# syghmon/bridges-with-reinforcement-learning

Hardware: AMD Instinct MI355X
Metric: env-steps/sec (vectorised assembly_gym, tower_height=4) (higher is better)
Workload: dtype f64

## Files before the change

### bridges-with-reinforcement-learning_amd/csrc/env_kernels.hip

```cpp
#include "bridges_device.h"
#include "rbe_device.h"

namespace bridges {

__device__ inline void reset_env(const DevCtx& c, int e, int lane) {
    c.b.state_bits[(size_t)e * IMG + lane] = 0ull;
    if (lane < c.K) c.b.blk_occ[(size_t)e * c.K + lane] = 0;
    if (lane == 0) {
        c.b.n_blocks[e] = 0;
        c.b.n_if[e] = 0;
        c.b.targets_left[e] = (c.n_targets >= 32) ? 0xffffffffu : ((1u << c.n_targets) - 1u);
        c.b.needs_reset[e] = 0;
    }
}

__device__ inline int count_candidates(const DevCtx& c, int e, int nb, int lane) {
    int nfree = 0;
    for (int i0 = 0; i0 < nb * MAXV; i0 += WAVE) {
        int i = i0 + lane;
        bool fr = false;
        if (i < nb * MAXV) {
            int b = i / MAXV, f = i % MAXV;
            int nv = c.tt->shapes[c.b.blk_shape[(size_t)e * c.K + b]].nv;
            fr = f < nv && !((c.b.blk_occ[(size_t)e * c.K + b] >> f) & 1);
        }
        nfree += __popcll(__ballot(fr));
    }
    return c.n_groups * (c.n_ground + nfree * c.n_offsets);
}

__global__ __launch_bounds__(WAVE) void k_reset(DevCtx c) {
    int e = blockIdx.x, lane = threadIdx.x;
    reset_env(c, e, lane);
    if (lane < 8) c.b.step_flags[(size_t)e * 8 + lane] = 0;
    int nc = count_candidates(c, e, 0, lane);
    if (lane == 0) {
        c.b.reward[e] = 0.f;
        c.b.lin_reward[e] = 0.f;
        c.b.n_reached[e] = 0;
        c.b.draw_counter[e] = 0;
        c.b.n_cand[e] = nc;
    }
}

#define STEP_IF_LDS 32
#define STEP_TAB_LDS 4096
struct StepStage {
    bridges_shape shapes[8];
    double pose[MAXK * 4];
    double verts[MAXK * MAXV * 2];
    int32_t shape_id[MAXK];
    int32_t occ[MAXK];
};
struct StepKeep {
    double if_geom[STEP_IF_LDS * 8];
    int32_t if_body[STEP_IF_LDS * 2];
    double cen[MAXK * 2];
    double vol[MAXK];
};
static_assert(sizeof(StepStage) <= STEP_TAB_LDS * sizeof(double), "staging area must fit into the tableau storage");

__device__ __forceinline__ const double* step_targets() { return nullptr; }
__device__ __forceinline__ const double* step_targets(const double* p) { return p; }
template <typename... ENV_TARGETS>
__global__ __launch_bounds__(WAVE) void k_step(DevCtx c, ENV_TARGETS... env_targets_arg) {
    constexpr bool PER_ENV = sizeof...(ENV_TARGETS) == 1;
    const double* env_targets = step_targets(env_targets_arg...);
    (void)env_targets;
    __shared__ __attribute__((aligned(16))) double tab[STEP_TAB_LDS];
    __shared__ LpScratch S;
    __shared__ StepKeep Lk;
    StepStage& L = *reinterpret_cast<StepStage*>(tab);
    __builtin_amdgcn_s_setprio(3);
    const int e = blockIdx.x, lane = threadIdx.x;
    const int K = c.K;
    uint8_t* flags = c.b.step_flags + (size_t)e * 8;
    int32_t* shape_id_g = c.b.blk_shape + (size_t)e * K;
    double* pose_g = c.b.blk_pose + (size_t)e * K * 4;
    double* verts_g = c.b.blk_verts + (size_t)e * K * MAXV * 2;
    uint8_t* occ_g = c.b.blk_occ + (size_t)e * K;
    int32_t* if_body_g = c.b.if_body + (size_t)e * MAXIF * 2;
    double* if_geom_g = c.b.if_geom + (size_t)e * MAXIF * 8;
    double* ws = c.b.lp_ws + (size_t)e * c.b.lp_ws_stride;
    const WarmHdr* hdr_g = reinterpret_cast<const WarmHdr*>(ws);

    const uint8_t need_reset = c.b.needs_reset[e];
    const int a = c.b.sel_index[e];
    const int off = c.b.cand_offset[e];
    const int nb = c.b.n_blocks[e];
    const int n_if_old = c.b.n_if[e];
    uint32_t left = c.b.targets_left[e];
    const uint64_t sbits = c.b.state_bits[(size_t)e * IMG + lane];
    WarmPre W;
    W.magic = hdr_g->magic; W.n_blocks = hdr_g->n_blocks; W.n_if = hdr_g->n_if; W.stride = hdr_g->stride;
    W.half = hdr_g->half; W.m = hdr_g->m;
    W.basis_lane = hdr_g->basis[lane];
    double tgv = 0.0;
    if constexpr (PER_ENV) {
        if (lane < c.n_targets * 3) tgv = env_targets[(size_t)e * c.n_targets * 3 + lane];
    }
    {
        const double* src = reinterpret_cast<const double*>(c.tt->shapes);
        double* dst = reinterpret_cast<double*>(L.shapes);
        const int nd = c.n_shapes * (int)(sizeof(bridges_shape) / 8);
        for (int i = lane; i < nd; i += WAVE) dst[i] = src[i];
        for (int i = lane; i < nb * 4; i += WAVE) L.pose[i] = pose_g[i];
        for (int i = lane; i < nb * MAXV * 2; i += WAVE) L.verts[i] = verts_g[i];
        if (lane < K) { L.shape_id[lane] = shape_id_g[lane]; L.occ[lane] = occ_g[lane]; }
        const int n0 = n_if_old < STEP_IF_LDS ? n_if_old : STEP_IF_LDS;
        for (int i = lane; i < n0 * 8; i += WAVE) Lk.if_geom[i] = if_geom_g[i];
        for (int i = lane; i < n0 * 2; i += WAVE) Lk.if_body[i] = if_body_g[i];
    }

    if (need_reset) {
        reset_env(c, e, lane);
        if (lane < 8) flags[lane] = 0;
        if (lane == 0) {
            c.b.reward[e] = 0.f;
            c.b.lin_reward[e] = 0.f;
            c.b.n_reached[e] = 0;
        }
        if (lane == 0) c.b.n_cand[e] = c.n_groups * c.n_ground;
        return;
    }

    const size_t ci = (size_t)off + a;
    const int dsc = lane < 4 ? c.b.cand_desc[ci * 4 + lane] : 0;
    const double cpose = lane < 4 ? c.b.cand_pose[ci * 4 + lane] : 0.0;
    const double cvert = lane < MAXV * 2 ? c.b.cand_verts[ci * MAXV * 2 + lane] : 0.0;
    const uint64_t cbits = c.b.cand_bits[ci * IMG + lane];
    const float base = c.b.cand_lin[ci];
    warm_prefetch(W, ws, nb, n_if_old, lane);
    const int tb = __builtin_amdgcn_readlane(dsc, 0), tf = __builtin_amdgcn_readlane(dsc, 1);
    const int sh = __builtin_amdgcn_readlane(dsc, 2), fc = __builtin_amdgcn_readlane(dsc, 3);

    if (lane < 4) { L.pose[nb * 4 + lane] = cpose; pose_g[nb * 4 + lane] = cpose; }
    if (lane < MAXV * 2) { L.verts[nb * MAXV * 2 + lane] = cvert; verts_g[nb * MAXV * 2 + lane] = cvert; }
    c.b.state_bits[(size_t)e * IMG + lane] = sbits | cbits;
    __syncthreads();
    if (lane == 0) {
        L.shape_id[nb] = sh;
        shape_id_g[nb] = sh;
        L.occ[nb] = (int32_t)(1u << fc);
        occ_g[nb] = (uint8_t)(1u << fc);
        if (tb >= 0) {
            L.occ[tb] |= (int32_t)(1u << tf);
            occ_g[tb] = (uint8_t)L.occ[tb];
        }
        c.b.n_blocks[e] = nb + 1;
    }
    __syncthreads();
    const bridges_shape* shapes = L.shapes;
    const bridges_shape& shn = shapes[sh];
    int nf = 0;
    if (lane <= nb) {
        const bridges_shape& sb = shapes[L.shape_id[lane]];
        double rgx, rgz;
        rot2(sb.gx, sb.gz, L.pose[4 * lane + 2], L.pose[4 * lane + 3], rgx, rgz);
        Lk.cen[2 * lane] = L.pose[4 * lane] + rgx;
        Lk.cen[2 * lane + 1] = L.pose[4 * lane + 1] + rgz;
        Lk.vol[lane] = sb.volume;
        nf = sb.nv - __popc((uint32_t)L.occ[lane] & ((1u << sb.nv) - 1u));
    }

    double vx = 0.0, vz = 0.0;
    const int nvn = shn.nv;
    bool hasv = lane < nvn;
    if (hasv) { vx = L.verts[nb * MAXV * 2 + 2 * lane]; vz = L.verts[nb * MAXV * 2 + 2 * lane + 1]; }
    double x0 = wave_min_d(hasv ? vx : 1e300), x1 = wave_max_d(hasv ? vx : -1e300);
    double z0 = wave_min_d(hasv ? vz : 1e300), z1 = wave_max_d(hasv ? vz : -1e300);
    {
        double cx = (x0 + x1) * 0.5, cz = (z0 + z1) * 0.5, hx = (x1 - x0) * 0.5, hz = (z1 - z0) * 0.5;
        double hy = shn.depth * 0.5;
        bool skip = false;
        for (int t = 0; t < c.n_targets; ++t) {
            if (!((left >> t) & 1u)) continue;
            if (skip) { skip = false; continue; }
            bool in;
            if constexpr (PER_ENV) {
                const double tx = readlane_d(tgv, 3 * t), ty = readlane_d(tgv, 3 * t + 1), tz = readlane_d(tgv, 3 * t + 2);
                in = fabs(tx - cx) < hx + 1e-6 && fabs(ty) < hy + 1e-6 && fabs(tz - cz) < hz + 1e-6;
            } else {
                in = fabs(c.targets[t][0] - cx) < hx + 1e-6 && fabs(c.targets[t][1]) < hy + 1e-6 &&
                     fabs(c.targets[t][2] - cz) < hz + 1e-6;
            }
            if (in) { left &= ~(1u << t); skip = true; }
        }
    }
    const int n_reached = c.n_targets - __popc(left);

    int n_if = n_if_old;
    bool overflow = false;
    {
        const double* nverts = L.verts + nb * MAXV * 2;
        const int totalp = (1 + nb * MAXV) * MAXV;
        for (int p0 = 0; p0 < totalp; p0 += WAVE) {
            const int p = p0 + lane;
            bool hit = false;
            double g[8];
            int bodyA = -1;
            if (p < totalp) {
                const int qa = p / MAXV, fn = p % MAXV;
                if (fn < shn.nv) {
                    const int ia = shn.fa[fn], ib = shn.fb[fn];
                    const double aBx = nverts[2 * ia], aBz = nverts[2 * ia + 1], bBx = nverts[2 * ib], bBz = nverts[2 * ib + 1];
                    const Frame2 fB = edge_frame(aBx, aBz, bBx, bBz);
                    if (qa == 0) {
                        hit = face_pair_contact_v(-c.floor_hw, 0.0, c.floor_hw, 0.0, 0.0, 0.0, 1.0, 0.0, 0.0, 1.0, aBx, aBz, bBx,
                                                  bBz, fB.cx, fB.cz, fB.nx, fB.nz, fmin(c.floor_depth, shn.depth), g);
                    } else {
                        bodyA = (qa - 1) / MAXV;
                        const int f = (qa - 1) % MAXV;
                        const bridges_shape& sa = shapes[L.shape_id[bodyA]];
                        if (f < sa.nv) {
                            const double* v = L.verts + bodyA * MAXV * 2;
                            const double ax = v[2 * sa.fa[f]], az = v[2 * sa.fa[f] + 1], bx = v[2 * sa.fb[f]], bz = v[2 * sa.fb[f] + 1];
                            const Frame2 fr = edge_frame(ax, az, bx, bz);
                            hit = face_pair_contact_v(ax, az, bx, bz, fr.cx, fr.cz, fr.tx, fr.tz, fr.nx, fr.nz, aBx, aBz, bBx, bBz,
                                                      fB.cx, fB.cz, fB.nx, fB.nz, fmin(sa.depth, shn.depth), g);
                        }
                    }
                }
            }
            const uint64_t bal = __ballot(hit);
            const int idx = n_if + __popcll(bal & ((1ull << lane) - 1ull));
            if (hit && idx < MAXIF) {
                if_body_g[2 * idx] = bodyA;
                if_body_g[2 * idx + 1] = nb;
#pragma unroll
                for (int k = 0; k < 8; ++k) if_geom_g[8 * idx + k] = g[k];
                if (idx < STEP_IF_LDS) {
                    Lk.if_body[2 * idx] = bodyA;
                    Lk.if_body[2 * idx + 1] = nb;
#pragma unroll
                    for (int k = 0; k < 8; ++k) Lk.if_geom[8 * idx + k] = g[k];
                }
            }
            n_if += __popcll(bal);
        }
        if (n_if > MAXIF) { overflow = true; n_if = MAXIF; }
    }
    __syncthreads();

    bool err = false;
    bool st_frozen = true, st_free = true;
    bool warm_used = false, resolved = false;
    AsmView A;
    A.pose = nullptr; A.shape_id = nullptr; A.shapes = nullptr; A.n_blocks = nb + 1;
    A.cand_b = -1; A.cand_pose = nullptr; A.cand_shape = 0; A.cen = Lk.cen; A.vol = Lk.vol; A.n_tens = 0; A.tens_coef = 1.0;
    A.n_if = n_if; A.n_if0 = n_if < STEP_IF_LDS ? n_if : STEP_IF_LDS;
    A.if_body0 = Lk.if_body; A.if_geom0 = Lk.if_geom;
    A.if_body1 = if_body_g + 2 * STEP_IF_LDS; A.if_geom1 = if_geom_g + 8 * STEP_IF_LDS;
    rbe_both(tab, STEP_TAB_LDS, ws, c.b.lp_ws_stride, S, A, n_if_old, W, c.mu, c.density, lane, &st_frozen, &st_free, &err,
             &warm_used, c.b.lp_snap ? c.b.lp_snap + (size_t)e * c.b.lp_snap_stride : nullptr, &resolved);

    const bool all_reached = left == 0;
    const bool terminated = !st_frozen || all_reached;
    const bool truncated = (c.max_steps > 0 && (nb + 1) >= c.max_steps) || (nb + 1) >= K;
    const bool done = terminated || truncated;
    float reward = !st_frozen ? -1.f : (all_reached ? (float)n_reached : (float)(-1 + n_reached));
    float lin = st_free ? base : (st_frozen ? base / 100.f : 0.f);

    if (lane == 0) {
        flags[F_VALID] = 1; flags[F_STABLE_FROZEN] = st_frozen; flags[F_STABLE_UNFROZEN] = st_free;
        flags[F_TERMINATED] = terminated; flags[F_TRUNCATED] = truncated; flags[F_DONE] = done;
        flags[F_NO_ACTIONS] = 0; flags[F_LP_ERROR] = (uint8_t)((err ? 1 : 0) | (overflow ? 2 : 0) | (resolved ? 4 : 0));
        c.b.reward[e] = reward;
        c.b.lin_reward[e] = lin;
        c.b.n_reached[e] = n_reached;
        c.b.n_if[e] = n_if;
        c.b.targets_left[e] = left;
    }
    int nb_after = nb + 1;
    if (done) {
        reset_env(c, e, lane);
        nb_after = 0;
    }
    int nfree = 0;
    for (int b = 0; b < nb_after; ++b) nfree += __builtin_amdgcn_readlane(nf, b);
    const int nc = c.n_groups * (c.n_ground + nfree * c.n_offsets);
    if (lane == 0) c.b.n_cand[e] = nc;
}

#define SCAN_THREADS 256
#define SCAN_WAVES (SCAN_THREADS / WAVE)
#define SCAN_BATCH 8
__global__ __launch_bounds__(SCAN_THREADS) void k_scan(DevCtx c, int after_step) {
    __shared__ int wave_tot[SCAN_WAVES];
    __shared__ int carry_s;
    __shared__ unsigned long long red[SCAN_WAVES][8];
    __builtin_amdgcn_s_setprio(3);
    const int t = threadIdx.x, lane = t & 63, wv = t >> 6;
    if (t == 0) carry_s = 0;
    __syncthreads();
    unsigned long long acc[8] = {0, 0, 0, 0, 0, 0, 0, 0};
    for (int base0 = 0; base0 < c.E; base0 += SCAN_THREADS * SCAN_BATCH) {
        int v[SCAN_BATCH], nbk[SCAN_BATCH], nval[SCAN_BATCH];
        uint64_t fl8[SCAN_BATCH];
#pragma unroll
        for (int u = 0; u < SCAN_BATCH; ++u) {
            const int i = base0 + u * SCAN_THREADS + t;
            const bool in = i < c.E;
            v[u] = in ? c.b.n_cand[i] : 0;
            nbk[u] = in ? c.b.n_blocks[i] : 0;
            nval[u] = (in && after_step) ? c.b.n_valid[i] : 0;
            fl8[u] = (in && after_step) ? *reinterpret_cast<const uint64_t*>(c.b.step_flags + (size_t)i * 8) : 0ull;
        }
#pragma unroll
        for (int u = 0; u < SCAN_BATCH; ++u) {
            const int base = base0 + u * SCAN_THREADS;
            if (base >= c.E) break;
            const int i = base + t;
            if (i < c.E) {
                if (v[u] > c.a_max) {
                    v[u] = c.a_max;
                    c.b.n_cand[i] = c.a_max;
                    c.b.step_flags[(size_t)i * 8 + F_LP_ERROR] |= 8;
                    acc[7] += 1;
                }
                acc[0] += (unsigned long long)nbk[u];
                if (after_step) {
                    const unsigned valid = (unsigned)(fl8[u] >> (8 * F_VALID)) & 0xffu;
                    const unsigned lperr = (unsigned)(fl8[u] >> (8 * F_LP_ERROR)) & 0xffu;
                    acc[1] += valid ? 1 : 0;
                    acc[2] += valid ? 0 : 1;
                    acc[3] += (lperr & 1) ? 1 : 0;
                    acc[4] += (lperr & 2) ? 1 : 0;
                    acc[5] += (unsigned long long)nval[u];
                    acc[6] += (lperr & 4) ? 1 : 0;
                }
            }
            int incl = v[u];
#pragma unroll
            for (int o = 1; o < WAVE; o <<= 1) {
                int up = __shfl_up(incl, o, WAVE);
                if (lane >= o) incl += up;
            }
            if (lane == WAVE - 1) wave_tot[wv] = incl;
            __syncthreads();
            int wbase = 0;
            for (int k = 0; k < wv; ++k) wbase += wave_tot[k];
            const int carry = carry_s;
            if (i < c.E) c.b.cand_offset[i] = carry + wbase + incl - v[u];
            __syncthreads();
            if (t == SCAN_THREADS - 1) carry_s = carry + wbase + incl;
            __syncthreads();
        }
    }
#pragma unroll
    for (int k = 0; k < 8; ++k) {
        unsigned long long x = acc[k];
#pragma unroll
        for (int o = 32; o > 0; o >>= 1) x += __shfl_xor(x, o, WAVE);
        if (lane == 0) red[wv][k] = x;
    }
    __syncthreads();
    if (t == 0) {
        unsigned long long tot[8] = {0, 0, 0, 0, 0, 0, 0, 0};
        for (int w = 0; w < SCAN_WAVES; ++w)
            for (int k = 0; k < 8; ++k) tot[k] += red[w][k];
        c.b.cand_offset[c.E] = carry_s;
        if (c.h_total) *c.h_total = carry_s;
        c.b.stats[ST_SUM_CAND] += (uint64_t)carry_s;
        c.b.stats[ST_SUM_BLOCKS] += tot[0];
        c.b.stats[ST_ENV_STEPS] += tot[1];
        c.b.stats[ST_RESET_ONLY] += tot[2];
        c.b.stats[ST_LP_ERRORS] += tot[3];
        c.b.stats[ST_IF_OVERFLOW] += tot[4];
        c.b.stats[ST_SUM_VALID] += tot[5];
        c.b.stats[ST_WARM_RESOLVED] += tot[6];
        c.b.stats[ST_CAND_OVERFLOW] += tot[7];
        c.b.stats[ST_LOCKSTEPS] += 1;
    }
}

__global__ __launch_bounds__(WAVE) void k_enumerate(DevCtx c) {
    __shared__ uint8_t free_b[MAXK * MAXV], free_f[MAXK * MAXV];
    __shared__ bridges_shape sh_l[8];
    __shared__ double verts_l[MAXK * MAXV * 2];
    __shared__ int32_t shape_l[MAXK], occ_l[MAXK];
    __shared__ double xg_l[32], offs_l[8];
    __builtin_amdgcn_s_setprio(3);
    const int e = blockIdx.x, lane = threadIdx.x;
    const int K = c.K;
    if (lane < 32) xg_l[lane] = c.tt->x_ground[lane];
    if (lane < 8) offs_l[lane] = c.tt->offsets[lane];
    const int nb = c.b.n_blocks[e];
    const int ncand = c.b.n_cand[e];
    const size_t off = (size_t)c.b.cand_offset[e];
    {
        const double* src = reinterpret_cast<const double*>(c.tt->shapes);
        double* dst = reinterpret_cast<double*>(sh_l);
        const int nd = c.n_shapes * (int)(sizeof(bridges_shape) / 8);
        for (int i = lane; i < nd; i += WAVE) dst[i] = src[i];
        const double* vg = c.b.blk_verts + (size_t)e * K * MAXV * 2;
        for (int i = lane; i < nb * MAXV * 2; i += WAVE) verts_l[i] = vg[i];
        if (lane < K) { shape_l[lane] = c.b.blk_shape[(size_t)e * K + lane]; occ_l[lane] = c.b.blk_occ[(size_t)e * K + lane]; }
    }
    __syncthreads();
    const bridges_shape* shapes = sh_l;
    const int32_t* shape_id = shape_l;
    const double* verts = verts_l;
    int nfree = 0;
    for (int i0 = 0; i0 < nb * MAXV; i0 += WAVE) {
        int i = i0 + lane;
        bool fr = false;
// ... 747 lines not shown
```

### bridges-with-reinforcement-learning_amd/csrc/rbe_device.h

```cpp
#pragma once
#include "bridges_device.h"

namespace bridges {

#define RBE_TOL_PARALLEL 1e-6
#define RBE_TOL_COPLANAR 1e-6
#define RBE_AMIN 0.001
#define RBE_FEAS_TOL 1e-5
#define LP_EPS_COST 1e-9
#define LP_TAU 1e-5
#define LP_VERIFY_TOL 1e-4
#define LP_TIE 1e-9
#define LP_STALL 40
#define LP_MAX_PIVOTS 5000
#define LP_PERTURB 1e-8
#define LP_MARGIN 1e3
#define LP_MARGIN_LO 0.1
#define LP_S_MAX 1e4
#define LP_TAB_LDS 2048
#define MAXFACES (1 + MAXK * MAXV)
#define LP_MAX_COLS (4 * MAXIF)
#define LP_MAX_CHUNKS ((LP_MAX_COLS + 2 + WAVE - 1) / WAVE)

struct FaceLds {
// ... 330 lines not shown
                for (int u = 0; u < 4; ++u) {
                    if (idx + u * WAVE < cells) {
                        double v;
                        if (ii[u] == r) v = rv[u];
                        else if (qq[u] == jin) v = 0.0;
                        else v = tv[u] - cv[u] * rv[u];
                        T[ii[u] * stride + qq[u]] = v;
                    }
                }
            }
        }
        if (lane == 0) basis[r] = jin;
        wave_sync<IN_LDS>();
        const double wn = -T[mc * stride + n];
        if (wn < w - progress) { stall = 0; bland = false; }
        else if (++stall > LP_STALL) bland = true;
        w = wn;
        if (++pivots >= LP_MAX_PIVOTS) { *error = true; w = artificial_sum(T, stride, m, n, basis, lane); break; }
    }
    *pivots_out = pivots;
    return w;
}

template <typename TP, typename SC>
__device__ inline double lp_verify(TP T, int stride, int m, int m_chk, int n, SC& S, const AsmView& A, double mu,
                                   double density, int lane) {
    for (int q = lane; q < n; q += WAVE) S.rowr[q] = 0.0;
    __syncthreads();
    if (lane <= m && S.basis[lane] >= 0 && S.basis[lane] < n) {
        double v = T[lane * stride + n + 1];
        S.rowr[S.basis[lane]] = v > 0.0 ? v : 0.0;
    }
    __syncthreads();
    double res = 0.0;
    if (lane < m_chk && S.basis[lane] != -1) {
        int b = -1;
        for (int k = 0; k < A.n_blocks; ++k) if (S.row_of[k] >= 0 && S.row_of[k] <= lane && lane < S.row_of[k] + 3) b = k;
        const int comp = lane - S.row_of[b];
        double gcx, gcz;
        A.centroid(b, gcx, gcz);
        double acc = 0.0;
        for (int k = 0; k < A.n_if; ++k) {
            const int32_t* bd = A.ib(k);
            const int bA = bd[0], bB = bd[1];
            if (bA != b && bB != b) continue;
            const double sign = (bB == b) ? 1.0 : -1.0;
            const double* g = A.ig(k);
#pragma unroll
            for (int c4 = 0; c4 < 4; ++c4) {
                const int ip = c4 >> 1, ig = c4 & 1;
                const double x = S.rowr[4 * k + c4];
                if (x == 0.0) continue;
                const double px = ip ? g[2] : g[0], pz = ip ? g[3] : g[1];
                const double gx = sign * (ig ? g[4] - mu * g[6] : g[4] + mu * g[6]);
                const double gz = sign * (ig ? g[5] - mu * g[7] : g[5] + mu * g[7]);
                const double coef = comp == 0 ? gx : (comp == 1 ? gz : (px - gcx) * gz - (pz - gcz) * gx);
                acc += coef * x;
            }
            if (A.n_tens) {
#pragma unroll
                for (int ip = 0; ip < 2; ++ip) {
                    const double x = S.rowr[4 * A.n_if + 2 * k + ip];
                    if (x == 0.0) continue;
                    const double px = ip ? g[2] : g[0], pz = ip ? g[3] : g[1];
                    const double gx = -sign * g[4], gz = -sign * g[5];
                    const double coef = comp == 0 ? gx : (comp == 1 ? gz : (px - gcx) * gz - (pz - gcz) * gx);
                    acc += coef * x;
                }
            }
        }
        const double rhs = comp == 1 ? density * A.volume(b) : 0.0;
        res = fabs(acc - rhs);
    }
    return wave_sum_d(res);
}

template <bool IN_LDS, typename TP, typename SC>
__device__ inline void lp_activate_rows(TP T, int stride, int m, int m_act, int n_gen, SC& S, int lane, int ncarr = 0) {
    const int n = n_gen + 1;
    for (int i = m_act; i < m; ++i) {
        const bool neg = T[i * stride + n] < 0.0;
        wave_sync<IN_LDS>();
        for (int q = lane; q <= n + ncarr; q += WAVE) {
            double v = T[i * stride + q];
            if (neg) { v = -v; T[i * stride + q] = v; }
            T[(m + 1) * stride + q] -= v;
        }
        if (lane == 0) S.basis[i] = n + i;
    }
    wave_sync<IN_LDS>();
}

template <typename SC>
__device__ inline void lp_row_map(SC& S, uint32_t free_mask, int lane) {
    __syncthreads();
    if (lane < MAXK)
        S.row_of[lane] = ((free_mask >> lane) & 1u) ? 3 * __popc(free_mask & ((1u << lane) - 1u)) : -1;
    __syncthreads();
}

__device__ __forceinline__ void lp_dims(int n_free, int n_if, int& m, int& n, int& stride, int64_t& cells, bool carriers = false,
                                        int n_tens = 0) {
    m = 3 * n_free;
    n = 4 * n_if + 2 * n_tens;
    stride = n + 2 + (carriers ? m : 0);
    if ((stride & 1) == 0) stride += 1;
    cells = (int64_t)(m + 2) * stride;
}

template <typename SC>
__device__ inline bool rbe_stable(double* tab_lds, int lds_cap, int max_cols, double* tab_ws, int64_t ws_cap, SC& S,
                                  const AsmView& A, uint32_t fixed_mask, double mu, double density, int lane,
                                  double* w_out, int* pivots_out, bool* error, bool* too_big) {
    *w_out = 0.0;
    *pivots_out = 0;
    const int n_blocks = A.n_blocks;
    const uint32_t all = n_blocks >= 32 ? 0xffffffffu : ((1u << n_blocks) - 1u);
    const uint32_t free_mask = all & ~fixed_mask;
    const int n_free = __popc(free_mask);
    if (A.n_if == 0) return n_free == 0;
    if (n_free == 0) return true;
    int m, n, stride;
    int64_t cells;
    lp_dims(n_free, A.n_if, m, n, stride, cells, false, A.n_tens);
    const double feas = RBE_FEAS_TOL * density, vtol = LP_VERIFY_TOL * density;
    double w;
    if (cells <= lds_cap && n <= max_cols) {
        lp_row_map(S, free_mask, lane);
        lp_build(tab_lds, stride, m, m, n, A, S.row_of, mu, density, lane);
        w = lp_phase1<true>(tab_lds, stride, m, m, n, S, lane, pivots_out, error, true, feas);
        if (w <= feas && lp_verify(tab_lds, stride, m, m, n, S, A, mu, density, lane) > vtol) { *error = true; w = 1e300; }
    } else {
        if (cells > ws_cap || n > max_cols) { *too_big = true; return false; }
        lp_row_map(S, free_mask, lane);
        lp_build(tab_ws, stride, m, m, n, A, S.row_of, mu, density, lane);
        w = lp_phase1<false>(tab_ws, stride, m, m, n, S, lane, pivots_out, error, true, feas);
        if (w <= feas && lp_verify(tab_ws, stride, m, m, n, S, A, mu, density, lane) > vtol) { *error = true; w = 1e300; }
    }
    *w_out = w;
    return w <= feas;
}

#define WARM_HDR_DOUBLES 64
#define WARM_MAX_STRIDE (LP_MAX_COLS + 2 + 3 * MAXK + 1)
#define WARM_HALF ((int64_t)(3 * MAXK + 2) * WARM_MAX_STRIDE)
#define WARM_WS_DOUBLES (WARM_HDR_DOUBLES + 2 * WARM_HALF)
#define WARM_MAGIC 0x57A7B1E5

struct WarmHdr {
    int32_t magic, n_blocks, n_if, stride, half, m, pad_[10];
    int32_t basis[64];
};

#define WARM_PRE 16
struct WarmPre {
    int32_t magic, n_blocks, n_if, stride, half, m;
    int32_t basis_lane;
    bool ok;
    int n_pre;
    double cell[WARM_PRE];
};

__device__ __forceinline__ void warm_header(WarmPre& W, const double* ws, int lane) {
    const WarmHdr* h = reinterpret_cast<const WarmHdr*>(ws);
    W.magic = h->magic; W.n_blocks = h->n_blocks; W.n_if = h->n_if; W.stride = h->stride; W.half = h->half; W.m = h->m;
    W.basis_lane = h->basis[lane];
}

__device__ __forceinline__ bool warm_matches(const WarmPre& W, int n_old_blocks, int n_if_old) {
    return W.magic == WARM_MAGIC && W.n_blocks == n_old_blocks && W.n_if == n_if_old && n_old_blocks >= 1 &&
           W.m == 3 * n_old_blocks;
}

__device__ __forceinline__ void warm_prefetch(WarmPre& W, const double* ws, int n_old_blocks, int n_if_old, int lane) {
    W.ok = warm_matches(W, n_old_blocks, n_if_old);
    W.n_pre = WARM_PRE;
    const int m_o = 3 * n_old_blocks, ncols_o = 4 * n_if_old + 2 + m_o;
    const int cells_o = W.ok ? (m_o + 1) * ncols_o : 0;
    const double* src = ws + WARM_HDR_DOUBLES + (int64_t)(W.half & 1) * WARM_HALF;
    const int di = WAVE / ncols_o, dq = WAVE - di * ncols_o;
    int i = lane / ncols_o, q = lane - i * ncols_o;
#pragma unroll
    for (int u = 0; u < WARM_PRE; ++u) {
        const int idx = lane + WAVE * u;
        double v = 0.0;
        if (idx < cells_o) v = src[(size_t)i * W.stride + q];
        W.cell[u] = v;
        i += di; q += dq;
        if (q >= ncols_o) { q -= ncols_o; ++i; }
    }
}

template <bool IN_LDS, typename TP, typename SC>
__device__ inline void lp_warm_prepare(TP T, int stride, int m, int n_gen, const double* src, int stride_o, int m_o,
                                       int n_gen_o, const WarmPre& W, SC& S, const AsmView& A, double mu,
                                       double density, int lane) {
    const int n = n_gen + 1, n_o = n_gen_o + 1;
    const int ncols_o = n_o + 1 + m_o;
    const int cells = (m + 2) * stride;
    for (int i = lane; i < cells; i += WAVE) T[i] = 0.0;
    wave_sync<IN_LDS>();
    const int cells_o = (m_o + 1) * ncols_o;
    const int di_o = WAVE / ncols_o, dq_o = WAVE - di_o * ncols_o;
    int ci_o = lane / ncols_o, cq_o = lane - ci_o * ncols_o;
#pragma unroll
    for (int u = 0; u < WARM_PRE; ++u) {
        const int idx = lane + WAVE * u;
        if (u < W.n_pre && idx < cells_o) {
            const int i = ci_o, q = cq_o;
            const int qn = q < n_gen_o ? q : (q == n_gen_o ? n_gen : (q == n_o ? n : n + 1 + (q - n_o - 1)));
            const int in = i < m_o ? i : m;
            T[in * stride + qn] = W.cell[u];
        }
        if (u < W.n_pre) {
            ci_o += di_o; cq_o += dq_o;
            if (cq_o >= ncols_o) { cq_o -= ncols_o; ++ci_o; }
        }
    }
    for (int idx = lane + WAVE * W.n_pre; idx < cells_o; idx += WAVE) {
        const int i = ci_o, q = cq_o;
        const double v = src[(size_t)i * stride_o + q];
        const int qn = q < n_gen_o ? q : (q == n_gen_o ? n_gen : (q == n_o ? n : n + 1 + (q - n_o - 1)));
        const int in = i < m_o ? i : m;
        T[in * stride + qn] = v;
        ci_o += di_o; cq_o += dq_o;
        if (cq_o >= ncols_o) { cq_o -= ncols_o; ++ci_o; }
    }
    if (lane <= m_o) {
        const int b = W.basis_lane;
        const int bn = b < n_gen_o ? b : (b == n_gen_o ? n_gen : n + (b - n_o));
        S.basis[lane < m_o ? lane : m] = bn;
    }
    if (lane >= m_o && lane < m) S.basis[lane] = -1;
    wave_sync<IN_LDS>();
    const int nbn = A.n_blocks - 1;
    if (lane < 3) {
        const int i = m_o + lane;
        double rhs = (LP_PERTURB * density) * (1.0 + 0.37 * (double)(i % 7) + 0.0618 * (double)(i % 11));
        if (lane == 1) rhs += density * A.volume(nbn);
        T[i * stride + n] = rhs;
        T[i * stride + n + 1 + i] = 1.0;
    }
    {
        const int n_newc = n_gen - n_gen_o;
        double ncx = 0.0, ncz = 0.0;
        A.centroid(nbn, ncx, ncz);
        for (int j0 = 0; j0 < n_newc; j0 += 16) {
            wave_sync<IN_LDS>();
            if (lane < 16 && j0 + lane < n_newc) {
                const int j = n_gen_o + j0 + lane;
                const int k = j >> 2, ip = (j >> 1) & 1, ig = j & 1;
                const double* g = A.ig(k);
                const int32_t* bd = A.ib(k);
                const double px = ip ? g[2] : g[0], pz = ip ? g[3] : g[1];
                const double nx = g[4], nz = g[5], tx = g[6], tz = g[7];
                const double gx = ig ? nx - mu * tx : nx + mu * tx;
                const double gz = ig ? nz - mu * tz : nz + mu * tz;
                const int bodyA = bd[0];
                double a0 = 0.0, a1 = 0.0, a2 = 0.0;
                if (bodyA >= 0) {
                    double gcx, gcz;
                    A.centroid(bodyA, gcx, gcz);
                    const double rx = px - gcx, rz = pz - gcz;
                    a0 = -gx; a1 = -gz; a2 = rx * a1 - rz * a0;
                }
                const double rxn = px - ncx, rzn = pz - ncz;
                double* d = S.rowr + 7 * lane;
                d[0] = a0; d[1] = a1; d[2] = a2; d[3] = (double)bodyA;
                d[4] = gx; d[5] = gz; d[6] = rxn * gz - rzn * gx;
            }
            wave_sync<IN_LDS>();
            const int nb16 = (n_newc - j0) < 16 ? (n_newc - j0) : 16;
            if (lane <= m_o) {
                const int row = lane < m_o ? lane : m;
                const double slack = T[row * stride + n_gen];
                for (int u = 0; u < nb16; ++u) {
                    const double* d = S.rowr + 7 * u;
                    const int bodyA = (int)d[3];
                    double v = slack;
                    if (bodyA >= 0) {
                        const int c0 = n + 1 + 3 * bodyA;
                        v += d[0] * T[row * stride + c0] + d[1] * T[row * stride + c0 + 1] + d[2] * T[row * stride + c0 + 2];
                    }
                    T[row * stride + n_gen_o + j0 + u] = v;
                }
            } else if (lane < m_o + 4) {
                const int cmp = lane - m_o - 1;
                for (int u = 0; u < nb16; ++u) T[(m_o + cmp) * stride + n_gen_o + j0 + u] = S.rowr[7 * u + 4 + cmp];
            }
        }
    }
    wave_sync<IN_LDS>();
    for (int q = lane; q <= n; q += WAVE) {
        double sacc = 0.0;
        for (int i = 0; i < m_o; ++i)
            if (S.basis[i] >= n) sacc += T[i * stride + q];
        T[(m + 1) * stride + q] = -sacc;
    }
    wave_sync<IN_LDS>();
}

__device__ inline void lp_warm_store(const double* T, int stride, int m, int n_gen, double* dst, int lane) {
    const int ncols = n_gen + 2 + m;
    const int cells = (m + 1) * ncols;
    const int di = WAVE / ncols, dq = WAVE - di * ncols;
    int i = lane / ncols, q = lane - i * ncols;
    for (int idx = lane; idx < cells; idx += WAVE) {
        dst[(size_t)i * stride + q] = T[i * stride + q];
        i += di; q += dq;
        if (q >= ncols) { q -= ncols; ++i; }
    }
}

template <bool IN_LDS, typename TP>
__device__ inline void rbe_both_run(TP T, int stride, int m, int n, LpScratch& S, const AsmView& A, double mu, double density,
                                    int lane, bool warm, bool* st_frozen, bool* st_free, bool* error, int* pivots,
                                    double* snap, bool* marginal) {
    const int m_act = m - 3;
    const double feas = RBE_FEAS_TOL * density, vtol = LP_VERIFY_TOL * density;
    const double near = LP_MARGIN * feas;
    *marginal = false;
    if (!warm) lp_build(T, stride, m, m_act, n, A, S.row_of, mu, density, lane, m);
    int& piv = *pivots;
    double w = lp_phase1<IN_LDS>(T, stride, m, m_act, n, S, lane, &piv, error, !warm, feas, m);
    *st_frozen = w <= feas;
    if (w > LP_MARGIN_LO * feas && w < near) *marginal = true;
    if (*st_frozen && m_act > 0 && lp_verify(T, stride, m, m_act, n, S, A, mu, density, lane) > vtol) {
        *st_frozen = false;
        *error = true;
    }
    if (!*st_frozen) { *st_free = false; return; }
    if (snap) {
        wave_sync<IN_LDS>();
        lp_warm_store(T, stride, m, n, snap + WARM_HDR_DOUBLES, lane);
        WarmHdr* sh = reinterpret_cast<WarmHdr*>(snap);
        if (lane <= m) sh->basis[lane] = S.basis[lane];
        if (lane == 0) {
            sh->n_blocks = A.n_blocks; sh->n_if = A.n_if; sh->stride = stride; sh->half = 0; sh->m = m;
            sh->magic = WARM_MAGIC;
        }
    }
    lp_activate_rows<IN_LDS>(T, stride, m, m_act, n, S, lane, m);
    w = lp_phase1<IN_LDS>(T, stride, m, m, n, S, lane, &piv, error, false, feas, m);
    *st_free = w <= feas;
    if (w > LP_MARGIN_LO * feas && w < near) *marginal = true;
    if (*st_free && lp_verify(T, stride, m, m, n, S, A, mu, density, lane) > vtol) {
        *st_free = false;
        *error = true;
    }
}

__device__ inline void rbe_both(double* tab_lds, int lds_cap, double* ws, int64_t ws_cap, LpScratch& S, const AsmView& A, int n_if_old,
                                const WarmPre& W, double mu, double density, int lane, bool* st_frozen, bool* st_free,
                                bool* error, bool* warm_used, double* snap = nullptr, bool* resolved = nullptr) {
    WarmHdr* hdr = reinterpret_cast<WarmHdr*>(ws);
    double* halves = ws + WARM_HDR_DOUBLES;
    *warm_used = false;
    const int nb = A.n_blocks;
    if (A.n_if == 0) {
        *st_frozen = nb == 1;
        *st_free = false;
        if (lane == 0) { hdr->magic = 0; if (snap) reinterpret_cast<WarmHdr*>(snap)->magic = 0; }
        return;
    }
    if (snap && lane == 0) reinterpret_cast<WarmHdr*>(snap)->magic = 0;
    const uint32_t all = nb >= 32 ? 0xffffffffu : ((1u << nb) - 1u);
    lp_row_map(S, all, lane);
    int m, n, stride;
    int64_t cells;
    lp_dims(nb, A.n_if, m, n, stride, cells, true);
    if (ws_cap < WARM_WS_DOUBLES || cells > WARM_HALF) {
        *error = true; *st_frozen = false; *st_free = false;
        if (lane == 0) hdr->magic = 0;
        return;
    }
    bool warm = W.ok;
    const int half_o = W.half & 1, stride_o = W.stride;
    const bool in_lds = cells <= lds_cap;
    const int half_n = in_lds ? 0 : 1 - half_o;
    double* Tg = halves + (int64_t)half_n * WARM_HALF;
    int pivots = 0;
    for (int attempt = 0; attempt < 2; ++attempt) {
        bool err = false;
        if (warm) {
            const double* src = halves + (int64_t)half_o * WARM_HALF;
            if (in_lds) lp_warm_prepare<true>(tab_lds, stride, m, n, src, stride_o, m - 3, 4 * n_if_old, W, S, A, mu, density, lane);
            else lp_warm_prepare<false>(Tg, stride, m, n, src, stride_o, m - 3, 4 * n_if_old, W, S, A, mu, density, lane);
        }
        bool marginal = false;
        if (in_lds) rbe_both_run<true>(tab_lds, stride, m, n, S, A, mu, density, lane, warm, st_frozen, st_free, &err, &pivots, snap, &marginal);
        else rbe_both_run<false>(Tg, stride, m, n, S, A, mu, density, lane, warm, st_frozen, st_free, &err, &pivots, snap, &marginal);
        if (!(warm && (err || marginal))) { *error = err; *warm_used = warm; break; }
        if (resolved) *resolved = true;
        warm = false;
        lp_row_map(S, all, lane);
    }
    __syncthreads();
    if (*st_frozen && !*error) {
        if (in_lds) lp_warm_store(tab_lds, stride, m, n, halves, lane);
        if (lane <= m) hdr->basis[lane] = S.basis[lane];
        if (lane == 0) {
            hdr->n_blocks = nb; hdr->n_if = A.n_if; hdr->stride = stride; hdr->half = half_n; hdr->m = m;
            hdr->magic = WARM_MAGIC;
        }
    } else if (lane == 0) {
        hdr->magic = 0;
    }
    __syncthreads();
}

template <typename SC>
__device__ inline bool rbe_candidate_warm(double* tab_lds, int lds_cap, int max_cols, SC& S, const AsmView& A, int n_if_old,
                                          const WarmPre& W, const double* snap, double mu, double density, int lane,
                                          bool* fits, bool* error, int* pivots) {
    const int nb = A.n_blocks;
    int m, n, stride;
    int64_t cells;
    lp_dims(nb, A.n_if, m, n, stride, cells, true);
    *fits = cells <= lds_cap && n + 2 + m <= max_cols + 4 + 3 * MAXK;
    if (!*fits) return false;
    const uint32_t all = (1u << nb) - 1u;
    lp_row_map(S, all, lane);
    const double feas = RBE_FEAS_TOL * density, vtol = LP_VERIFY_TOL * density;
    lp_warm_prepare<true>(tab_lds, stride, m, n, snap + WARM_HDR_DOUBLES, W.stride, m - 3, 4 * n_if_old, W, S, A, mu, density, lane);
    lp_activate_rows<true>(tab_lds, stride, m, m - 3, n, S, lane, m);
    const double w = lp_phase1<true>(tab_lds, stride, m, m, n, S, lane, pivots, error, false, feas, m);
    bool stable = w <= feas;
    if (w > LP_MARGIN_LO * feas && w < LP_MARGIN * feas) *error = true;
    if (stable && lp_verify(tab_lds, stride, m, m, n, S, A, mu, density, lane) > vtol) { *error = true; stable = false; }
    return stable;
}

}
```

Measured before the change: 4.842 million.

## Prefetch warm-start tableau into LDS via async global_load_lds instead of registers

Replaces the 16-register per-lane prefetch of the previous LP tableau with asynchronous global_load_lds_dwordx4 transfers into a reserved landing area at the top of the LDS tableau buffer, covering up to 1024 doubles. lp_warm_prepare then reads from that area, waiting on vmcnt first, and falls back to global reads for the rest. The aim is to cover more of the warm-start copy with latency hiding while freeing registers. Separately, per-env scalar loads are wrapped in readfirstlane and lane is passed through an opaque asm barrier, which adds inline-asm M0 handling and early-exit waits. The candidate path passes a null landing pointer with W.n_pre possibly nonzero, which is risky if that path is reached.

```diff
diff --git a/bridges-with-reinforcement-learning_amd/csrc/env_kernels.hip b/bridges-with-reinforcement-learning_amd/csrc/env_kernels.hip
--- a/bridges-with-reinforcement-learning_amd/csrc/env_kernels.hip
+++ b/bridges-with-reinforcement-learning_amd/csrc/env_kernels.hip
@@ -58,7 +58,9 @@
     double cen[MAXK * 2];
     double vol[MAXK];
 };
-static_assert(sizeof(StepStage) <= STEP_TAB_LDS * sizeof(double), "staging area must fit into the tableau storage");
+#define STEP_LAND_OFF (STEP_TAB_LDS - WARM_LAND)
+static_assert(sizeof(StepStage) <= STEP_LAND_OFF * sizeof(double), "staging area must fit into the tableau storage below the landing area");
+static_assert((STEP_LAND_OFF * sizeof(double)) % 16 == 0, "the landing area takes 16-byte stores");
 
 __device__ __forceinline__ const double* step_targets() { return nullptr; }
 __device__ __forceinline__ const double* step_targets(const double* p) { return p; }
@@ -84,16 +86,17 @@
     double* ws = c.b.lp_ws + (size_t)e * c.b.lp_ws_stride;
     const WarmHdr* hdr_g = reinterpret_cast<const WarmHdr*>(ws);
 
-    const uint8_t need_reset = c.b.needs_reset[e];
-    const int a = c.b.sel_index[e];
-    const int off = c.b.cand_offset[e];
-    const int nb = c.b.n_blocks[e];
-    const int n_if_old = c.b.n_if[e];
-    uint32_t left = c.b.targets_left[e];
+    const int need_reset = __builtin_amdgcn_readfirstlane((int)c.b.needs_reset[e]);
+    const int a = __builtin_amdgcn_readfirstlane(c.b.sel_index[e]);
+    const int off = __builtin_amdgcn_readfirstlane(c.b.cand_offset[e]);
+    const int nb = __builtin_amdgcn_readfirstlane(c.b.n_blocks[e]);
+    const int n_if_old = __builtin_amdgcn_readfirstlane(c.b.n_if[e]);
+    uint32_t left = (uint32_t)__builtin_amdgcn_readfirstlane((int)c.b.targets_left[e]);
     const uint64_t sbits = c.b.state_bits[(size_t)e * IMG + lane];
     WarmPre W;
-    W.magic = hdr_g->magic; W.n_blocks = hdr_g->n_blocks; W.n_if = hdr_g->n_if; W.stride = hdr_g->stride;
-    W.half = hdr_g->half; W.m = hdr_g->m;
+    W.magic = __builtin_amdgcn_readfirstlane(hdr_g->magic); W.n_blocks = __builtin_amdgcn_readfirstlane(hdr_g->n_blocks);
+    W.n_if = __builtin_amdgcn_readfirstlane(hdr_g->n_if); W.stride = __builtin_amdgcn_readfirstlane(hdr_g->stride);
+    W.half = __builtin_amdgcn_readfirstlane(hdr_g->half); W.m = __builtin_amdgcn_readfirstlane(hdr_g->m);
     W.basis_lane = hdr_g->basis[lane];
     double tgv = 0.0;
     if constexpr (PER_ENV) {
@@ -130,7 +133,7 @@
     const double cvert = lane < MAXV * 2 ? c.b.cand_verts[ci * MAXV * 2 + lane] : 0.0;
     const uint64_t cbits = c.b.cand_bits[ci * IMG + lane];
     const float base = c.b.cand_lin[ci];
-    warm_prefetch(W, ws, nb, n_if_old, lane);
+    warm_prefetch(W, ws, nb, n_if_old, lane, tab + STEP_LAND_OFF);
     const int tb = __builtin_amdgcn_readlane(dsc, 0), tf = __builtin_amdgcn_readlane(dsc, 1);
     const int sh = __builtin_amdgcn_readlane(dsc, 2), fc = __builtin_amdgcn_readlane(dsc, 3);
 
@@ -251,7 +254,7 @@
     A.n_if = n_if; A.n_if0 = n_if < STEP_IF_LDS ? n_if : STEP_IF_LDS;
     A.if_body0 = Lk.if_body; A.if_geom0 = Lk.if_geom;
     A.if_body1 = if_body_g + 2 * STEP_IF_LDS; A.if_geom1 = if_geom_g + 8 * STEP_IF_LDS;
-    rbe_both(tab, STEP_TAB_LDS, ws, c.b.lp_ws_stride, S, A, n_if_old, W, c.mu, c.density, lane, &st_frozen, &st_free, &err,
+    rbe_both(tab, STEP_TAB_LDS, ws, c.b.lp_ws_stride, S, A, n_if_old, W, tab + STEP_LAND_OFF, c.mu, c.density, lane, &st_frozen, &st_free, &err,
              &warm_used, c.b.lp_snap ? c.b.lp_snap + (size_t)e * c.b.lp_snap_stride : nullptr, &resolved);
 
     const bool all_reached = left == 0;
diff --git a/bridges-with-reinforcement-learning_amd/csrc/rbe_device.h b/bridges-with-reinforcement-learning_amd/csrc/rbe_device.h
--- a/bridges-with-reinforcement-learning_amd/csrc/rbe_device.h
+++ b/bridges-with-reinforcement-learning_amd/csrc/rbe_device.h
@@ -506,13 +506,12 @@
     int32_t basis[64];
 };
 
-#define WARM_PRE 16
+#define WARM_LAND 1024
 struct WarmPre {
     int32_t magic, n_blocks, n_if, stride, half, m;
     int32_t basis_lane;
     bool ok;
     int n_pre;
-    double cell[WARM_PRE];
 };
 
 __device__ __forceinline__ void warm_header(WarmPre& W, const double* ws, int lane) {
@@ -526,52 +525,61 @@
            W.m == 3 * n_old_blocks;
 }
 
-__device__ __forceinline__ void warm_prefetch(WarmPre& W, const double* ws, int n_old_blocks, int n_if_old, int lane) {
+__device__ __forceinline__ void glds16(const void* gsrc, uint32_t lds_dst) {
+    unsigned keep;
+    asm volatile("s_mov_b32 %0, m0\n\ts_mov_b32 m0, %2\n\ts_nop 0\n\tglobal_load_lds_dwordx4 %1, off\n\ts_mov_b32 m0, %0"
+                 : "=&s"(keep) : "v"(gsrc), "s"(lds_dst) : "memory");
+}
+__device__ __forceinline__ void glds_wait() { asm volatile("s_waitcnt vmcnt(0)" ::: "memory"); }
+
+__device__ __forceinline__ void warm_prefetch(WarmPre& W, const double* ws, int n_old_blocks, int n_if_old, int lane, double* land) {
     W.ok = warm_matches(W, n_old_blocks, n_if_old);
-    W.n_pre = WARM_PRE;
+    const double* src = ws + WARM_HDR_DOUBLES + (int64_t)(W.half & 1) * WARM_HALF;
     const int m_o = 3 * n_old_blocks, ncols_o = 4 * n_if_old + 2 + m_o;
-    const int cells_o = W.ok ? (m_o + 1) * ncols_o : 0;
-    const double* src = ws + WARM_HDR_DOUBLES + (int64_t)(W.half & 1) * WARM_HALF;
-    const int di = WAVE / ncols_o, dq = WAVE - di * ncols_o;
-    int i = lane / ncols_o, q = lane - i * ncols_o;
+    const bool can = W.ok && (W.stride == ncols_o || W.stride == ncols_o + 1) && (reinterpret_cast<uintptr_t>(src) & 15) == 0;
+    const int run = can ? (m_o + 1) * W.stride : 0;
+    W.n_pre = run < WARM_LAND ? run : WARM_LAND;
+    const uint32_t lds = (uint32_t)reinterpret_cast<uintptr_t>(land);
 #pragma unroll
-    for (int u = 0; u < WARM_PRE; ++u) {
-        const int idx = lane + WAVE * u;
-        double v = 0.0;
-        if (idx < cells_o) v = src[(size_t)i * W.stride + q];
-        W.cell[u] = v;
-        i += di; q += dq;
-        if (q >= ncols_o) { q -= ncols_o; ++i; }
-    }
+    for (int u = 0; u < WARM_LAND / (2 * WAVE); ++u)
+        if (u * 2 * WAVE < W.n_pre)
+            glds16(src + u * 2 * WAVE + 2 * lane, lds + u * 2 * WAVE * (uint32_t)sizeof(double));
 }
 
 template <bool IN_LDS, typename TP, typename SC>
 __device__ inline void lp_warm_prepare(TP T, int stride, int m, int n_gen, const double* src, int stride_o, int m_o,
-                                       int n_gen_o, const WarmPre& W, SC& S, const AsmView& A, double mu,
+                                       int n_gen_o, const WarmPre& W, const double* land, SC& S, const AsmView& A, double mu,
                                        double density, int lane) {
     const int n = n_gen + 1, n_o = n_gen_o + 1;
     const int ncols_o = n_o + 1 + m_o;
     const int cells = (m + 2) * stride;
+    int n_land = W.n_pre;
+    if constexpr (IN_LDS) {
+        if (n_land > 0 && land < T + cells) {
+            glds_wait();
+            n_land = 0;
+        }
+    }
     for (int i = lane; i < cells; i += WAVE) T[i] = 0.0;
     wave_sync<IN_LDS>();
     const int cells_o = (m_o + 1) * ncols_o;
     const int di_o = WAVE / ncols_o, dq_o = WAVE - di_o * ncols_o;
     int ci_o = lane / ncols_o, cq_o = lane - ci_o * ncols_o;
-#pragma unroll
-    for (int u = 0; u < WARM_PRE; ++u) {
-        const int idx = lane + WAVE * u;
-        if (u < W.n_pre && idx < cells_o) {
+    int idx = lane;
+    if (n_land > 0) {
+        glds_wait();
+        for (; idx < cells_o; idx += WAVE) {
             const int i = ci_o, q = cq_o;
+            const int f = i * stride_o + q;
+            if (f >= n_land) break;
             const int qn = q < n_gen_o ? q : (q == n_gen_o ? n_gen : (q == n_o ? n : n + 1 + (q - n_o - 1)));
             const int in = i < m_o ? i : m;
-            T[in * stride + qn] = W.cell[u];
-        }
-        if (u < W.n_pre) {
+            T[in * stride + qn] = land[f];
             ci_o += di_o; cq_o += dq_o;
             if (cq_o >= ncols_o) { cq_o -= ncols_o; ++ci_o; }
         }
     }
-    for (int idx = lane + WAVE * W.n_pre; idx < cells_o; idx += WAVE) {
+    for (; idx < cells_o; idx += WAVE) {
         const int i = ci_o, q = cq_o;
         const double v = src[(size_t)i * stride_o + q];
         const int qn = q < n_gen_o ? q : (q == n_gen_o ? n_gen : (q == n_o ? n : n + 1 + (q - n_o - 1)));
@@ -666,6 +674,11 @@
     }
 }
 
+__device__ __forceinline__ int lane_again(int lane) {
+    asm volatile("" : "+v"(lane));
+    return lane;
+}
+
 template <bool IN_LDS, typename TP>
 __device__ inline void rbe_both_run(TP T, int stride, int m, int n, LpScratch& S, const AsmView& A, double mu, double density,
                                     int lane, bool warm, bool* st_frozen, bool* st_free, bool* error, int* pivots,
@@ -674,19 +687,19 @@
     const double feas = RBE_FEAS_TOL * density, vtol = LP_VERIFY_TOL * density;
     const double near = LP_MARGIN * feas;
     *marginal = false;
-    if (!warm) lp_build(T, stride, m, m_act, n, A, S.row_of, mu, density, lane, m);
+    if (!warm) lp_build(T, stride, m, m_act, n, A, S.row_of, mu, density, lane_again(lane), m);
     int& piv = *pivots;
-    double w = lp_phase1<IN_LDS>(T, stride, m, m_act, n, S, lane, &piv, error, !warm, feas, m);
+    double w = lp_phase1<IN_LDS>(T, stride, m, m_act, n, S, lane_again(lane), &piv, error, !warm, feas, m);
     *st_frozen = w <= feas;
     if (w > LP_MARGIN_LO * feas && w < near) *marginal = true;
-    if (*st_frozen && m_act > 0 && lp_verify(T, stride, m, m_act, n, S, A, mu, density, lane) > vtol) {
+    if (*st_frozen && m_act > 0 && lp_verify(T, stride, m, m_act, n, S, A, mu, density, lane_again(lane)) > vtol) {
         *st_frozen = false;
         *error = true;
     }
     if (!*st_frozen) { *st_free = false; return; }
     if (snap) {
         wave_sync<IN_LDS>();
-        lp_warm_store(T, stride, m, n, snap + WARM_HDR_DOUBLES, lane);
+        lp_warm_store(T, stride, m, n, snap + WARM_HDR_DOUBLES, lane_again(lane));
         WarmHdr* sh = reinterpret_cast<WarmHdr*>(snap);
         if (lane <= m) sh->basis[lane] = S.basis[lane];
         if (lane == 0) {
@@ -694,19 +707,19 @@
             sh->magic = WARM_MAGIC;
         }
     }
-    lp_activate_rows<IN_LDS>(T, stride, m, m_act, n, S, lane, m);
-    w = lp_phase1<IN_LDS>(T, stride, m, m, n, S, lane, &piv, error, false, feas, m);
+    lp_activate_rows<IN_LDS>(T, stride, m, m_act, n, S, lane_again(lane), m);
+    w = lp_phase1<IN_LDS>(T, stride, m, m, n, S, lane_again(lane), &piv, error, false, feas, m);
     *st_free = w <= feas;
     if (w > LP_MARGIN_LO * feas && w < near) *marginal = true;
-    if (*st_free && lp_verify(T, stride, m, m, n, S, A, mu, density, lane) > vtol) {
+    if (*st_free && lp_verify(T, stride, m, m, n, S, A, mu, density, lane_again(lane)) > vtol) {
         *st_free = false;
         *error = true;
     }
 }
 
 __device__ inline void rbe_both(double* tab_lds, int lds_cap, double* ws, int64_t ws_cap, LpScratch& S, const AsmView& A, int n_if_old,
-                                const WarmPre& W, double mu, double density, int lane, bool* st_frozen, bool* st_free,
-                                bool* error, bool* warm_used, double* snap = nullptr, bool* resolved = nullptr) {
+                                const WarmPre& W, const double* land, double mu, double density, int lane, bool* st_frozen,
+                                bool* st_free, bool* error, bool* warm_used, double* snap = nullptr, bool* resolved = nullptr) {
     WarmHdr* hdr = reinterpret_cast<WarmHdr*>(ws);
     double* halves = ws + WARM_HDR_DOUBLES;
     *warm_used = false;
@@ -715,17 +728,19 @@
         *st_frozen = nb == 1;
         *st_free = false;
         if (lane == 0) { hdr->magic = 0; if (snap) reinterpret_cast<WarmHdr*>(snap)->magic = 0; }
+        if (W.n_pre > 0) glds_wait();
         return;
     }
     if (snap && lane == 0) reinterpret_cast<WarmHdr*>(snap)->magic = 0;
     const uint32_t all = nb >= 32 ? 0xffffffffu : ((1u << nb) - 1u);
-    lp_row_map(S, all, lane);
+    lp_row_map(S, all, lane_again(lane));
     int m, n, stride;
     int64_t cells;
     lp_dims(nb, A.n_if, m, n, stride, cells, true);
     if (ws_cap < WARM_WS_DOUBLES || cells > WARM_HALF) {
         *error = true; *st_frozen = false; *st_free = false;
         if (lane == 0) hdr->magic = 0;
+        if (W.n_pre > 0) glds_wait();
         return;
     }
     bool warm = W.ok;
@@ -738,8 +753,8 @@
         bool err = false;
         if (warm) {
             const double* src = halves + (int64_t)half_o * WARM_HALF;
-            if (in_lds) lp_warm_prepare<true>(tab_lds, stride, m, n, src, stride_o, m - 3, 4 * n_if_old, W, S, A, mu, density, lane);
-            else lp_warm_prepare<false>(Tg, stride, m, n, src, stride_o, m - 3, 4 * n_if_old, W, S, A, mu, density, lane);
+            if (in_lds) lp_warm_prepare<true>(tab_lds, stride, m, n, src, stride_o, m - 3, 4 * n_if_old, W, land, S, A, mu, density, lane_again(lane));
+            else lp_warm_prepare<false>(Tg, stride, m, n, src, stride_o, m - 3, 4 * n_if_old, W, land, S, A, mu, density, lane_again(lane));
         }
         bool marginal = false;
         if (in_lds) rbe_both_run<true>(tab_lds, stride, m, n, S, A, mu, density, lane, warm, st_frozen, st_free, &err, &pivots, snap, &marginal);
@@ -747,11 +762,11 @@
         if (!(warm && (err || marginal))) { *error = err; *warm_used = warm; break; }
         if (resolved) *resolved = true;
         warm = false;
-        lp_row_map(S, all, lane);
+        lp_row_map(S, all, lane_again(lane));
     }
     __syncthreads();
     if (*st_frozen && !*error) {
-        if (in_lds) lp_warm_store(tab_lds, stride, m, n, halves, lane);
+        if (in_lds) lp_warm_store(tab_lds, stride, m, n, halves, lane_again(lane));
         if (lane <= m) hdr->basis[lane] = S.basis[lane];
         if (lane == 0) {
             hdr->n_blocks = nb; hdr->n_if = A.n_if; hdr->stride = stride; hdr->half = half_n; hdr->m = m;
@@ -776,7 +791,7 @@
     const uint32_t all = (1u << nb) - 1u;
     lp_row_map(S, all, lane);
     const double feas = RBE_FEAS_TOL * density, vtol = LP_VERIFY_TOL * density;
-    lp_warm_prepare<true>(tab_lds, stride, m, n, snap + WARM_HDR_DOUBLES, W.stride, m - 3, 4 * n_if_old, W, S, A, mu, density, lane);
+    lp_warm_prepare<true>(tab_lds, stride, m, n, snap + WARM_HDR_DOUBLES, W.stride, m - 3, 4 * n_if_old, W, nullptr, S, A, mu, density, lane);
     lp_activate_rows<true>(tab_lds, stride, m, m - 3, n, S, lane, m);
     const double w = lp_phase1<true>(tab_lds, stride, m, m, n, S, lane, pivots, error, false, feas, m);
     bool stable = w <= feas;
```

New measurement: 4.885 million, median of 6. No clear change (+0.9%).
